# BioinfoMachineLearning/bio-diffusion

Hardware: NVIDIA H100
Metric: molecules/sec (1000-step sample) (higher is better)
Workload: dtype bf16x2 (split hi+lo operands, f32 accumulate; <=1e-4 of the fp32 reference)

## Files before the change

bio-diffusion_b200/csrc/bdiff_layers_tc.cu:

```cuda
#include "bdiff_node_tc.cuh"

namespace bdiff {

__device__ __forceinline__ int ld_acquire_gpu(const int* p) {
  int v;
  asm volatile("ld.acquire.gpu.global.s32 %0, [%1];" : "=r"(v) : "l"(p) : "memory");
  return v;
}
__device__ __forceinline__ void st_release_gpu(int* p, int v) {
  asm volatile("st.release.gpu.global.s32 [%0], %1;" ::"l"(p), "r"(v) : "memory");
}

union LayersTail {
  TcBars bars;
  EdgeTail edge;
  NodeTail node;
};
constexpr size_t LAYERS_SMEM_BYTES = XE_BLOCKS * (size_t)X_BLOCK + TC_NSLOT * (size_t)TC_SLOT + sizeof(LayersTail) + 1024;
static_assert(LAYERS_SMEM_BYTES + 64 <= 232448, "shared memory budget of the layer megakernel (227 KiB per block)");

constexpr int LAYERS_THREADS = 384;
constexpr int LAYERS_REG_COMPUTE = 232, LAYERS_REG_SERVICE = 40;
static_assert(256 * LAYERS_REG_COMPUTE + 128 * LAYERS_REG_SERVICE <= 168 * LAYERS_THREADS, "setmaxnreg pool");
constexpr int RING_CONSUMERS = TC_EPI / 32;

template <int NS, int NU, class Issue>
__device__ __forceinline__ void run_seg(TcBars& B, uint32_t raddr, uint32_t& ci, int nch, int scol, bool sfresh, int ucol,
                                        bool ufresh, Issue&& issue) {
  constexpr int RS = NS ? NS / 2 : 1, RU = NU ? NU / 2 : 1;
  const int wg = threadIdx.x >> 7;
  const bool lead = (threadIdx.x & 31) == 0;
  for (int h = 0; h < 2; ++h) {
    float s[RS], u[RU];
    if (NS) {
      if (sfresh) {
#pragma unroll
        for (int i = 0; i < RS; ++i) s[i] = 0.f;
      } else {
        acc_load<NS>(s, scol + h * NS, wg);
      }
    }
    if (NU) {
      if (ufresh) {
#pragma unroll
        for (int i = 0; i < RU; ++i) u[i] = 0.f;
      } else {
        acc_load<NU>(u, ucol + h * NU, wg);
      }
    }
    for (int c = 0; c < nch; ++c) {
      const uint32_t slot = ci % TC_NSLOT;
      float ts[RS], tu[RU];
#pragma unroll
      for (int i = 0; i < RS; ++i) ts[i] = 0.f;
#pragma unroll
      for (int i = 0; i < RU; ++i) tu[i] = 0.f;
      mbar_wait(&B.full[slot], (ci / TC_NSLOT) & 1);
      wgmma_fence();
      issue(ts, tu, raddr + slot * TC_SLOT, c);
      wgmma_commit();
      wgmma_wait<0>();
      acc_fence<RS>(ts);
      acc_fence<RU>(tu);
      mbar_arrive_if(&B.empty[slot], lead);
      ++ci;
      if (NS) {
#pragma unroll
        for (int i = 0; i < RS; ++i) s[i] += ts[i];
      }
      if (NU) {
#pragma unroll
        for (int i = 0; i < RU; ++i) u[i] += tu[i];
      }
    }
    if (NS) acc_store<NS>(s, scol + h * NS, wg);
    if (NU) acc_store<NU>(u, ucol + h * NU, wg);
  }
}

template <int ED, int XD>
__global__ void __launch_bounds__(LAYERS_THREADS, 1) k_layers_tc(Plan p, Dims d, EmbedW ew, LayerSched q, Work w) {
  constexpr int HID0 = (64 + XD) / 4;
  constexpr int H2 = HID0 / 2;
  constexpr int K0RAW = ED + HID0 + 9;
  constexpr int K0S = (K0RAW + 15) / 16;
  static_assert(HID0 % 2 == 0 && H2 * 3 <= 32 && HID0 + 9 <= 32 && ED % 16 == 0, "layout");

  extern __shared__ unsigned char smem_raw[];
  unsigned char* smem = smem_raw + ((1024u - (smem_u32(smem_raw) & 1023u)) & 1023u);
  unsigned char* X = smem;
  unsigned char* ring = smem + XE_BLOCKS * X_BLOCK;
  unsigned char* tail = ring + TC_NSLOT * TC_SLOT;
  TcBars& B = *reinterpret_cast<TcBars*>(tail);
  const int tid = threadIdx.x, warp = __shfl_sync(0xffffffffu, tid >> 5, 0), lane = tid & 31;
  const int hid0 = d.hid0;
  const int per_layer = q.TE + q.TN;
  const int total_items = q.nitems;
  int* const flags = q.sched + 2;

  if (tid == 0) {
    for (int i = 0; i < TC_NSLOT; ++i) { mbar_init(&B.full[i], 1); mbar_init(&B.empty[i], RING_CONSUMERS); }
    for (int i = 0; i < 2; ++i) { mbar_init(&B.item_full[i], 1); mbar_init(&B.item_empty[i], TC_EPI + 1); }
    mbar_init(&B.tile_done, TC_EPI);
    mbar_init(&B.wbar, 1);
    mbar_fence_init();
    tm_base = w.acc + (size_t)blockIdx.x * TM_COLS * 128;
  }
  __syncthreads();

  if (warp == 8) {
    asm volatile("setmaxnreg.dec.sync.aligned.u32 %0;\n" ::"n"(LAYERS_REG_SERVICE));
    if (lane == 0) {
      uint32_t ci = 0;
      for (uint32_t k = 0;; ++k) {
        const uint32_t slot = k & 1;
        mbar_wait_backoff(&B.item_empty[slot], ((k >> 1) & 1) ^ 1);
        int type = -1, layer = 0, tile = 0;
        for (;;) {
          const int qi = atomicAdd(q.sched, 1);
          if (qi >= 2 * total_items) break;
          const int it = __ldg(q.items + (qi >> 1));
          type = (it >> 30) & 1; layer = (it >> 24) & 63; tile = 2 * (it & 0xffffff) + (qi & 1);
          if (tile < (type == 0 ? q.TE : q.TN)) break;
          type = -1;
        }
        B.item[slot][0] = type; B.item[slot][1] = layer; B.item[slot][2] = tile;
        mbar_arrive(&B.item_full[slot]);
        if (type < 0) break;
        const size_t stride = type == 0 ? q.edge_blob_stride : q.node_blob_stride;
// ... 87 lines not shown
            cp(s.wgp, lw.Wgp, 256); cp(s.bgp, lw.bgp, 1);
            if (!last) {
              cp(s.u.nx.b0, wn.b0, 256);
              cp(s.u.nx.Wd0i, wn.Wd0i, 32 * hid0); cp(s.u.nx.Wd0j, wn.Wd0j, 32 * hid0);
              cp(s.u.nx.Wf0i, wn.Wf0i, 96); cp(s.u.nx.Wf0j, wn.Wf0j, 96);
            } else {
              cp(s.u.pj.pWd, ew.pWd, 32 * 32); cp(s.u.pj.pWf, ew.pWf, 96); cp(s.u.pj.pbs, ew.pbs, d.Hin);
            }
          }
        }
        mbar_wait(&B.wbar, pw);
        pw ^= 1;
        cur_type = type; cur_layer = layer;
      }
      if (tid == 0) {
        int lo = 0, hi = -1;
        const int* fbase = flags;
        if (type == 0) {
          if (layer > 0) {
            const int2 dep = q.edge_dep[tile];
            lo = dep.x; hi = dep.y;
            fbase = flags + (size_t)(layer - 1) * per_layer + q.TE;
          }
        } else {
          const int2 dep = q.node_dep[tile];
          lo = dep.x; hi = dep.y;
          fbase = flags + (size_t)layer * per_layer;
        }
        const long long t0 = clock64();
        for (int u = lo; u <= hi; ++u) {
          while (ld_acquire_gpu(fbase + u) == 0) {
            if (clock64() - t0 > (1ll << 32)) { atomicExch(q.err, 1); __threadfence_system(); __trap(); }
          }
        }
      }
      named_bar_sync(3, TC_EPI);
      __threadfence();
      if (tid == 0 && w.dbg && k < 16) w.dbg[(size_t)blockIdx.x * 64 + 4 * k + 2] = clock64();
      es = 0;
      stamp = nullptr;
      if (w.dbg && k >= 2 && !stamped[type]) { stamp = w.dbg + 256 * 64 + (size_t)blockIdx.x * 64 + type * 32; stamped[type] = true; }
      PH();
      const int last = type == 1 && layer == q.L - 1;
      int ph = 0;
      auto gemm = [&](int phase) __attribute__((always_inline)) {
        if (type == 0) {
          const int ph = phase;
#include "edge_tile_mma.inc"
        } else {
          const int ph = phase;
#include "node_r4_tile_mma.inc"
        }
      };
      auto publish = [&]() __attribute__((always_inline)) { fence_proxy_async(); named_bar_sync(3, TC_EPI); PH(); gemm(ph++); named_bar_sync(3, TC_EPI); PH(); };
      auto wait_d = [&]() __attribute__((always_inline)) {};
      auto release_u = [&]() __attribute__((always_inline)) { named_bar_sync(3, TC_EPI); gemm(-1); named_bar_sync(3, TC_EPI); };
      if (type == 0) {
        EdgeTail& T = *reinterpret_cast<EdgeTail*>(tail);
        const int half = tid >> 7, r = tid & 127;
        const SmallW& sw = T.sw;
        (void)release_u;
#include "edge_tile_epilogue.inc"
      } else {
        NodeTail& T = *reinterpret_cast<NodeTail*>(tail);
        NodeScratch& SC = *reinterpret_cast<NodeScratch*>(X + R5_BLOCKS * R5_BLOCK);
        const int l = lane, s = warp, c0 = warp * 32;
        const SmallWR4& sw = T.sw;
        (void)T;
#include "node_r4_tile_epilogue.inc"
      }
      PH();
      if (tid == 0 && w.dbg && k < 16) w.dbg[(size_t)blockIdx.x * 64 + 4 * k + 3] = clock64();
      mbar_arrive(&B.tile_done);
      mbar_arrive(&B.item_empty[slot]);
    }
  }
  __syncthreads();
}

bool tc_supported(int Ed, int Xd) { return (Ed == 64 && Xd == 16) || (Ed == 16 && Xd == 8); }

cudaError_t tc_layers_configure() {
  cudaError_t e = cudaFuncSetAttribute(k_layers_tc<64, 16>, cudaFuncAttributeMaxDynamicSharedMemorySize,
                                       (int)LAYERS_SMEM_BYTES);
  if (e != cudaSuccess) return e;
  return cudaFuncSetAttribute(k_layers_tc<16, 8>, cudaFuncAttributeMaxDynamicSharedMemorySize, (int)LAYERS_SMEM_BYTES);
}

void launch_layers_tc(cudaStream_t st, const Plan& p, const Dims& d, const EmbedW& ew, const LayerSched& q,
                      const Work& w, int num_sms) {
  const int grid = 2 * q.nitems < num_sms ? 2 * q.nitems : num_sms;
  if (d.Ed == 64) k_layers_tc<64, 16><<<grid, LAYERS_THREADS, LAYERS_SMEM_BYTES, st>>>(p, d, ew, q, w);
  else k_layers_tc<16, 8><<<grid, LAYERS_THREADS, LAYERS_SMEM_BYTES, st>>>(p, d, ew, q, w);
}

}
```

bio-diffusion_b200/csrc/bdiff_tc.cuh:

```cuda
#pragma once
#include <cuda_bf16.h>
#include <stdint.h>

#include "bdiff_common.cuh"

namespace bdiff {

__device__ __forceinline__ uint32_t sw128_offset(int r, int k) {
  return (uint32_t)(r * 128 + ((((k >> 3) ^ (r & 7)) & 7) << 4) + (k & 7) * 2);
}

__device__ __forceinline__ uint64_t gmma_desc_sw128(uint32_t saddr) {
  uint64_t d = 0;
  d |= (uint64_t)((saddr >> 4) & 0x3FFF);
  d |= (uint64_t)1 << 16;
  d |= (uint64_t)((1024 >> 4) & 0x3FFF) << 32;
  d |= (uint64_t)1 << 62;
  return d;
}

__device__ __forceinline__ uint64_t gmma_desc_k16(uint32_t saddr, uint32_t lbo, uint32_t sbo) {
  uint64_t d = 0;
  d |= (uint64_t)((saddr >> 4) & 0x3FFF);
  d |= (uint64_t)((lbo >> 4) & 0x3FFF) << 16;
// ... 4 lines not shown
template <int SA>
__device__ __forceinline__ void wgmma_n128(float* d, uint64_t ad, uint64_t bd) {
  asm volatile(
      "{\n.reg .pred p;\nsetp.ne.b32 p, %66, 0;\n"
      "wgmma.mma_async.sync.aligned.m64n128k16.f32.bf16.bf16 "
      "{%0,%1,%2,%3,%4,%5,%6,%7,%8,%9,%10,%11,%12,%13,%14,%15,%16,%17,%18,%19,%20,%21,%22,%23,%24,%25,%26,%27,%28,%29,%30,%31,%32,%33,%34,%35,%36,%37,%38,%39,%40,%41,%42,%43,%44,%45,%46,%47,%48,%49,%50,%51,%52,%53,%54,%55,%56,%57,%58,%59,%60,%61,%62,%63}, %64, %65, p, %67, 1, 0, 0;\n}\n"
      : "+f"(d[0]), "+f"(d[1]), "+f"(d[2]), "+f"(d[3]), "+f"(d[4]), "+f"(d[5]), "+f"(d[6]), "+f"(d[7]), "+f"(d[8]), "+f"(d[9]), "+f"(d[10]), "+f"(d[11]), "+f"(d[12]), "+f"(d[13]), "+f"(d[14]), "+f"(d[15]), "+f"(d[16]), "+f"(d[17]), "+f"(d[18]), "+f"(d[19]), "+f"(d[20]), "+f"(d[21]), "+f"(d[22]), "+f"(d[23]), "+f"(d[24]), "+f"(d[25]), "+f"(d[26]), "+f"(d[27]), "+f"(d[28]), "+f"(d[29]), "+f"(d[30]), "+f"(d[31]), "+f"(d[32]), "+f"(d[33]), "+f"(d[34]), "+f"(d[35]), "+f"(d[36]), "+f"(d[37]), "+f"(d[38]), "+f"(d[39]), "+f"(d[40]), "+f"(d[41]), "+f"(d[42]), "+f"(d[43]), "+f"(d[44]), "+f"(d[45]), "+f"(d[46]), "+f"(d[47]), "+f"(d[48]), "+f"(d[49]), "+f"(d[50]), "+f"(d[51]), "+f"(d[52]), "+f"(d[53]), "+f"(d[54]), "+f"(d[55]), "+f"(d[56]), "+f"(d[57]), "+f"(d[58]), "+f"(d[59]), "+f"(d[60]), "+f"(d[61]), "+f"(d[62]), "+f"(d[63])
      : "l"(ad), "l"(bd), "r"(1), "n"(SA));
}

template <int SA>
__device__ __forceinline__ void wgmma_n32(float* d, uint64_t ad, uint64_t bd) {
  asm volatile(
      "{\n.reg .pred p;\nsetp.ne.b32 p, %18, 0;\n"
      "wgmma.mma_async.sync.aligned.m64n32k16.f32.bf16.bf16 "
      "{%0,%1,%2,%3,%4,%5,%6,%7,%8,%9,%10,%11,%12,%13,%14,%15}, %16, %17, p, %19, 1, 0, 0;\n}\n"
      : "+f"(d[0]), "+f"(d[1]), "+f"(d[2]), "+f"(d[3]), "+f"(d[4]), "+f"(d[5]), "+f"(d[6]), "+f"(d[7]), "+f"(d[8]), "+f"(d[9]), "+f"(d[10]), "+f"(d[11]), "+f"(d[12]), "+f"(d[13]), "+f"(d[14]), "+f"(d[15])
      : "l"(ad), "l"(bd), "r"(1), "n"(SA));
}

template <int SA>
__device__ __forceinline__ void wgmma_n16(float* d, uint64_t ad, uint64_t bd) {
  asm volatile(
      "{\n.reg .pred p;\nsetp.ne.b32 p, %10, 0;\n"
      "wgmma.mma_async.sync.aligned.m64n16k16.f32.bf16.bf16 "
      "{%0,%1,%2,%3,%4,%5,%6,%7}, %8, %9, p, %11, 1, 0, 0;\n}\n"
      : "+f"(d[0]), "+f"(d[1]), "+f"(d[2]), "+f"(d[3]), "+f"(d[4]), "+f"(d[5]), "+f"(d[6]), "+f"(d[7])
      : "l"(ad), "l"(bd), "r"(1), "n"(SA));
}

__device__ __forceinline__ void wgmma_fence() { asm volatile("wgmma.fence.sync.aligned;" ::: "memory"); }
__device__ __forceinline__ void wgmma_commit() { asm volatile("wgmma.commit_group.sync.aligned;" ::: "memory"); }
template <int N>
__device__ __forceinline__ void wgmma_wait() { asm volatile("wgmma.wait_group.sync.aligned %0;" ::"n"(N) : "memory"); }
template <int R>
__device__ __forceinline__ void acc_fence(float* d) {
#pragma unroll
  for (int i = 0; i < R; ++i) asm volatile("" : "+f"(d[i])::"memory");
}

__device__ __forceinline__ void fence_proxy_async() { asm volatile("fence.proxy.async.shared::cta;" ::: "memory"); }
__device__ __forceinline__ void mbar_arrive(uint64_t* bar) {
  asm volatile("mbarrier.arrive.shared::cta.b64 _, [%0];" ::"r"(smem_u32(bar)) : "memory");
}
__device__ __forceinline__ void mbar_arrive_if(uint64_t* bar, bool pred) {
  asm volatile("{\n.reg .pred p;\nsetp.ne.b32 p, %1, 0;\n@p mbarrier.arrive.shared::cta.b64 _, [%0];\n}\n" ::"r"(smem_u32(bar)),
               "r"((int)pred) : "memory");
}

__shared__ float* tm_base;
__device__ __forceinline__ float* tm_word(uint32_t taddr) {
  return tm_base + (size_t)(taddr & 0xffffu) * 128 + (taddr >> 16) + (threadIdx.x & 31);
}
template <int N>
__device__ __forceinline__ void acc_store(const float* d, int col0, int wg) {
  const int lane = threadIdx.x & 31, row = 64 * wg + 16 * ((threadIdx.x >> 5) & 3) + (lane >> 2);
#pragma unroll
  for (int j = 0; j < N / 2; ++j)
    tm_base[(size_t)(col0 + 8 * (j >> 2) + 2 * (lane & 3) + (j & 1)) * 128 + row + 8 * ((j >> 1) & 1)] = d[j];
}
template <int N>
__device__ __forceinline__ void acc_load(float* d, int col0, int wg) {
  const int lane = threadIdx.x & 31, row = 64 * wg + 16 * ((threadIdx.x >> 5) & 3) + (lane >> 2);
#pragma unroll
  for (int j = 0; j < N / 2; ++j)
    d[j] = tm_base[(size_t)(col0 + 8 * (j >> 2) + 2 * (lane & 3) + (j & 1)) * 128 + row + 8 * ((j >> 1) & 1)];
}

__device__ __forceinline__ void tmem_ld8_nw(uint32_t taddr, uint32_t* r) {
  const float* p = tm_word(taddr);
#pragma unroll
  for (int i = 0; i < 8; ++i) r[i] = __float_as_uint(p[i * 128]);
}
__device__ __forceinline__ void tmem_ld32_nw(uint32_t taddr, uint32_t* r) {
  const float* p = tm_word(taddr);
#pragma unroll
  for (int i = 0; i < 32; ++i) r[i] = __float_as_uint(p[i * 128]);
}
__device__ __forceinline__ void tmem_ld_wait() {}
__device__ __forceinline__ void tmem_ld8(uint32_t taddr, float* v) {
  const float* p = tm_word(taddr);
#pragma unroll
  for (int i = 0; i < 8; ++i) v[i] = p[i * 128];
}
__device__ __forceinline__ void tmem_ld32(uint32_t taddr, float* v) {
  const float* p = tm_word(taddr);
#pragma unroll
  for (int i = 0; i < 32; ++i) v[i] = p[i * 128];
}
__device__ __forceinline__ void tmem_st8_nw(uint32_t taddr, const float* v) {
  float* p = tm_word(taddr);
#pragma unroll
  for (int i = 0; i < 8; ++i) p[i * 128] = v[i];
}
__device__ __forceinline__ void tmem_st_wait() {}
template <int N8>
__device__ __forceinline__ void tmem_ld8xN(uint32_t taddr, float* v) {
  const float* p = tm_word(taddr);
#pragma unroll
  for (int i = 0; i < N8 * 8; ++i) v[i] = p[i * 128];
}
template <int N8>
__device__ __forceinline__ void tmem_st8xN(uint32_t taddr, const float* v) {
#pragma unroll
  for (int q = 0; q < N8; ++q) tmem_st8_nw(taddr + q * 8, v + q * 8);
}
__device__ __forceinline__ void tmem_ld64(uint32_t taddr, float* v) { tmem_ld8xN<8>(taddr, v); }
__device__ __forceinline__ void tmem_st8(uint32_t taddr, const float* v) { tmem_st8_nw(taddr, v); }
__device__ __forceinline__ void tc_fence_before() {}
__device__ __forceinline__ void tc_fence_after() {}

#if defined(__CUDA_ARCH__) && __CUDA_ARCH__ < 1000
__device__ __forceinline__ float2 __fmul2_rn(float2 a, float2 b) { return make_float2(a.x * b.x, a.y * b.y); }
__device__ __forceinline__ float2 __fadd2_rn(float2 a, float2 b) { return make_float2(a.x + b.x, a.y + b.y); }
__device__ __forceinline__ float2 __ffma2_rn(float2 a, float2 b, float2 c) { return make_float2(fmaf(a.x, b.x, c.x), fmaf(a.y, b.y, c.y)); }
#endif

__device__ __forceinline__ float tanh_fast(float x) {
  float y;
// ... 77 lines not shown
```

bio-diffusion_b200/csrc/edge_tile_epilogue.inc:

```
      const long long g = (long long)tile * TMT + r;
      constexpr int PV = HID0 * 3 + 9, PF4 = (PV + 3) / 4, PLD = PF4 * 4 + 1;
      constexpr int XF4 = XD * 3 / 4, XLD = XD * 3 + 1;
      static_assert(K0S <= 8 && TMT * XLD * 4 <= 2 * X_BLOCK && TMT * PLD * 4 <= 3 * X_BLOCK, "staging areas");
      float* sFx = reinterpret_cast<float*>(X + 2 * X_BLOCK);
      float* sFp = reinterpret_cast<float*>(X + 6 * X_BLOCK);
      const int4 rc = __ldg(p.edge_rc + g);
      float f[9];
      {
        constexpr int F4_ROW = ED / 4;
        const float4* eb = reinterpret_cast<const float4*>(w.e + (size_t)tile * TMT * ED);
        const float4* xb = reinterpret_cast<const float4*>(w.xi + (size_t)tile * TMT * XD * 3);
        float4 ev[TMT * F4_ROW / TC_EPI], xv[TMT * XF4 / TC_EPI];
#pragma unroll
        for (int i = 0; i < TMT * F4_ROW / TC_EPI; ++i) ev[i] = eb[i * TC_EPI + tid];
#pragma unroll
        for (int i = 0; i < TMT * XF4 / TC_EPI; ++i) xv[i] = xb[i * TC_EPI + tid];
#pragma unroll
        for (int qq = 0; qq < 9; ++qq) f[qq] = w.frames[(size_t)g * 9 + qq];
        if (half == 0) { T.sRow[r] = rc.x; T.sCol[r] = rc.y; T.sB[r] = rc.z; T.sNa[r] = rc.w; }
#pragma unroll
        for (int i = 0; i < TMT * F4_ROW / TC_EPI; ++i) {
          const int idx = i * TC_EPI + tid;
          const int rr = idx / F4_ROW, kk = (idx % F4_ROW) * 4;
          xe_store4(X, rr, kk, ev[i].x, ev[i].y, ev[i].z, ev[i].w);
        }
#pragma unroll
        for (int i = 0; i < TMT * XF4 / TC_EPI; ++i) {
          const int idx = i * TC_EPI + tid;
          float* dst = sFx + (idx / XF4) * XLD + (idx % XF4) * 4;
          dst[0] = xv[i].x; dst[1] = xv[i].y; dst[2] = xv[i].z; dst[3] = xv[i].w;
        }
      }
      const int row = rc.x;
      const float* pi = w.PI + (size_t)(row < 0 ? 0 : row) * kPStride;
      named_bar_sync(3, TC_EPI);
      {
        float4 pv[(TMT * PF4 + TC_EPI - 1) / TC_EPI];
#pragma unroll
        for (int i = 0; i < (TMT * PF4 + TC_EPI - 1) / TC_EPI; ++i) {
          const int idx = i * TC_EPI + tid;
          pv[i] = make_float4(0.f, 0.f, 0.f, 0.f);
          if (idx < TMT * PF4) {
            const int rr = idx / PF4, cj = T.sCol[rr];
            if (cj >= 0) pv[i] = *reinterpret_cast<const float4*>(w.PJ + (size_t)cj * kPStride + kH + (idx - rr * PF4) * 4);
          }
        }
        float vdh[32], vdf0[9];
#pragma unroll
        for (int i = 0; i < 32; ++i) vdh[i] = 0.f;
#pragma unroll
        for (int i = 0; i < 9; ++i) vdf0[i] = 0.f;
        if (row >= 0) {
#pragma unroll
          for (int i = 0; i < H2 * 3; ++i) vdh[i] = pi[kH + half * H2 * 3 + i];
          if (half == 0) {
#pragma unroll
            for (int i = 0; i < 9; ++i) vdf0[i] = pi[kH + HID0 * 3 + i];
          }
        }
        float xi[XD * 3];
#pragma unroll
        for (int c = 0; c < XD * 3; ++c) xi[c] = sFx[r * XLD + c];
#pragma unroll
        for (int i = 0; i < (TMT * PF4 + TC_EPI - 1) / TC_EPI; ++i) {
          const int idx = i * TC_EPI + tid;
          if (idx < TMT * PF4) {
            const int rr = idx / PF4;
            float* dst = sFp + rr * PLD + (idx - rr * PF4) * 4;
            dst[0] = pv[i].x; dst[1] = pv[i].y; dst[2] = pv[i].z; dst[3] = pv[i].w;
          }
        }
        named_bar_sync(3, TC_EPI);
        const float* pjv = sFp + r * PLD;
#pragma unroll
        for (int i = 0; i < H2 * 3; ++i) vdh[i] += pjv[half * H2 * 3 + i];
        if (half == 0) {
#pragma unroll
          for (int i = 0; i < 9; ++i) vdf0[i] += pjv[HID0 * 3 + i];
        }
#pragma unroll
        for (int c = 0; c < XD; ++c) {
#pragma unroll
          for (int h = 0; h < H2; ++h) {
            const float wd = sw.Wd0x[c * HID0 + half * H2 + h];
            vdh[h * 3 + 0] = fmaf(wd, xi[c * 3 + 0], vdh[h * 3 + 0]);
            vdh[h * 3 + 1] = fmaf(wd, xi[c * 3 + 1], vdh[h * 3 + 1]);
            vdh[h * 3 + 2] = fmaf(wd, xi[c * 3 + 2], vdh[h * 3 + 2]);
          }
        }
#pragma unroll
        for (int h = 0; h < H2; ++h)
          xe_store1(X, r, ED + half * H2 + h, safe_norm3(vdh[h * 3], vdh[h * 3 + 1], vdh[h * 3 + 2]));
        tmem_st8xN<4>(tl + TM_VD0 + half * 32, vdh);
        tmem_st_wait();
        if (half == 0) {
#pragma unroll
          for (int c = 0; c < XD; ++c)
#pragma unroll
            for (int ch = 0; ch < 3; ++ch) {
              const float wf = sw.Wf0x[c * 3 + ch];
              vdf0[ch * 3 + 0] = fmaf(wf, xi[c * 3 + 0], vdf0[ch * 3 + 0]);
              vdf0[ch * 3 + 1] = fmaf(wf, xi[c * 3 + 1], vdf0[ch * 3 + 1]);
              vdf0[ch * 3 + 2] = fmaf(wf, xi[c * 3 + 2], vdf0[ch * 3 + 2]);
            }
#pragma unroll
          for (int ch = 0; ch < 3; ++ch)
#pragma unroll
            for (int ax = 0; ax < 3; ++ax)
              xe_store1(X, r, ED + HID0 + ch * 3 + ax,
                        f[ax * 3] * vdf0[ch * 3] + f[ax * 3 + 1] * vdf0[ch * 3 + 1] + f[ax * 3 + 2] * vdf0[ch * 3 + 2]);
#pragma unroll
          for (int i = HID0 + 9; i < K0S * 16 - ED; ++i) xe_store1(X, r, ED + i, 0.f);
        }
      }
      publish();

      {
        float4 pa[8];
        float pj[32];
        const int colj = rc.y;
        const int cjn = colj < 0 ? 0 : colj;
        const float* pjt = w.PJT + ((size_t)(cjn >> 5) * 256 + half * 128) * 32 + (cjn & 31);
        auto prefetch = [&](int c) {
          const float* pc = pjt + c * 1024;
#pragma unroll
          for (int i = 0; i < 32; ++i) pj[i] = pc[i * 32];
#pragma unroll
          for (int qq = 0; qq < 8; ++qq) pa[qq] = *reinterpret_cast<const float4*>(pi + half * 128 + c * 32 + qq * 4);
        };
        prefetch(0);
        wait_d();
        for (int c = 0; c < 4; ++c) {
          const int c0 = half * 128 + c * 32;
          float v[32];
          tmem_ld32(tl + TM_S + c0, v);
#pragma unroll
          for (int qq = 0; qq < 8; ++qq) {
            v[qq * 4 + 0] += pa[qq].x + pj[qq * 4 + 0]; v[qq * 4 + 1] += pa[qq].y + pj[qq * 4 + 1];
            v[qq * 4 + 2] += pa[qq].z + pj[qq * 4 + 2]; v[qq * 4 + 3] += pa[qq].w + pj[qq * 4 + 3];
          }
          if (c < 3) prefetch(c + 1);
#pragma unroll
          for (int qq = 0; qq < 16; ++qq) {
            const float2 p0 = silu_acc2(make_float2(v[2 * qq], v[2 * qq + 1]));
            v[2 * qq] = p0.x; v[2 * qq + 1] = p0.y;
          }
#pragma unroll
          for (int qq = 0; qq < 4; ++qq) xe_store8(X, r, c0 + qq * 8, v + qq * 8);
        }
      }
      publish();

      float vd[24], vdf[9];
      float2 adot2 = make_float2(0.f, 0.f);
      for (int k = 1; k <= 3; ++k) {
        wait_d();
        float part[33], other[33];
        if (k == 1) {
          float vd0[HID0 * 3];
          {
            float t0[64];
            float* t1 = t0 + 32;
            tmem_ld64(tl + TM_VD0, t0);
#pragma unroll
            for (int i = 0; i < H2 * 3; ++i) { vd0[i] = t0[i]; vd0[H2 * 3 + i] = t1[i]; }
          }
          tc_fence_before();
          named_bar_sync(3, TC_EPI);
          tc_fence_after();
          gate_update<HID0, true, false>(tl, half, TM_U0, vd0, sw.Wu0, sw.bg[0], sw.Wdk[0], sw.Wfk[0], part);
        } else {
          gate_update<8, false, false>(tl, half, ((k - 1) & 1) ? TM_U1 : TM_U0, vd, sw.Wuk[k - 2], sw.bg[k - 1],
                                       sw.Wdk[k - 1], sw.Wfk[k - 1], part);
        }
        pair_exchange33(tl, half, part, other);
#pragma unroll
        for (int i = 0; i < 24; ++i) vd[i] = half == 0 ? part[i] + other[i] : other[i] + part[i];
#pragma unroll
        for (int i = 0; i < 9; ++i) vdf[i] = half == 0 ? part[24 + i] + other[24 + i] : other[24 + i] + part[24 + i];
        {
          float a[16];
          if (half == 0) {
#pragma unroll
            for (int h = 0; h < 8; ++h) a[h] = safe_norm3(vd[h * 3], vd[h * 3 + 1], vd[h * 3 + 2]);
#pragma unroll
            for (int i = 0; i < 8; ++i) {
              const int ch = i / 3, ax = i - ch * 3;
              a[8 + i] = f[ax * 3] * vdf[ch * 3] + f[ax * 3 + 1] * vdf[ch * 3 + 1] + f[ax * 3 + 2] * vdf[ch * 3 + 2];
            }
          } else {
            a[0] = f[6] * vdf[6] + f[7] * vdf[7] + f[8] * vdf[8];
#pragma unroll
            for (int i = 1; i < 16; ++i) a[i] = 0.f;
          }
          xe_store8_extra(X, r, half * 16, a);
          xe_store8_extra(X, r, half * 16 + 8, a + 8);
        }
        publish();
        wait_d();
        if (k < 3 && half == 0) {
          float z[32];
#pragma unroll
          for (int i = 0; i < 32; ++i) z[i] = 0.f;
          tmem_st8xN<4>(tl + (((k + 1) & 1) ? TM_U1 : TM_U0), z);
          tmem_st_wait();
        }
        for (int c0 = half * 128; c0 < half * 128 + 128; c0 += 64) {
          float v[64];
          tmem_ld64(tl + TM_S + c0, v);
#pragma unroll
          for (int qq = 0; qq < 8; ++qq) {
            float m[8];
            xe_load8(X, r, c0 + qq * 8, m);
            const float4 b0 = *reinterpret_cast<const float4*>(&sw.bk[k - 1][c0 + qq * 8]);
            const float4 b1 = *reinterpret_cast<const float4*>(&sw.bk[k - 1][c0 + qq * 8 + 4]);
            const float2 bb[4] = {make_float2(b0.x, b0.y), make_float2(b0.z, b0.w), make_float2(b1.x, b1.y),
                                  make_float2(b1.z, b1.w)};
            float2 mm[4];
#pragma unroll
            for (int i = 0; i < 4; ++i)
              mm[i] = __fadd2_rn(make_float2(m[2 * i], m[2 * i + 1]),
                                 silu_acc2(__fadd2_rn(make_float2(v[qq * 8 + 2 * i], v[qq * 8 + 2 * i + 1]), bb[i])));
#pragma unroll
            for (int i = 0; i < 4; ++i) { m[2 * i] = mm[i].x; m[2 * i + 1] = mm[i].y; }
            xe_store8(X, r, c0 + qq * 8, m);
            if (k == 3) {
              const float4 w0 = *reinterpret_cast<const float4*>(&sw.wa[c0 + qq * 8]);
              const float4 w1 = *reinterpret_cast<const float4*>(&sw.wa[c0 + qq * 8 + 4]);
              adot2 = __ffma2_rn(mm[0], make_float2(w0.x, w0.y), adot2);
              adot2 = __ffma2_rn(mm[1], make_float2(w0.z, w0.w), adot2);
              adot2 = __ffma2_rn(mm[2], make_float2(w1.x, w1.y), adot2);
              adot2 = __ffma2_rn(mm[3], make_float2(w1.z, w1.w), adot2);
            }
          }
        }
        if (k == 3) T.sAttn[half][r] = adot2.x + adot2.y;
        publish();
      }
      const int wr0 = warp * 16;
      uint32_t m_start, m_end;
      {
        const int li = lane & 15, tr = wr0 + li;
        const int rw = T.sRow[tr];
        const int rp = tr > 0 ? T.sRow[tr - 1] : -2;
        const int rn = tr < TMT - 1 ? T.sRow[tr + 1] : -2;
        m_start = __ballot_sync(0xffffffffu, rw != rp) & 0xffffu;
        m_end = __ballot_sync(0xffffffffu, rw != rn && rw >= 0) & 0xffffu;
        if (lane == 0) T.winfo[warp] = m_start | (m_end << 16);
      }
      named_bar_sync(3, TC_EPI);
      const bool cutL = T.sB[0] != 0;
      const bool cutR = T.sRow[TMT - 1] >= 0 && T.sB[TMT - 1] != T.sNa[TMT - 1] - 1;
      const bool cont_in = !(m_start & 1u);
      float attw[16];
#pragma unroll
      for (int i = 0; i < 16; ++i) attw[i] = sigmoid_acc(T.sAttn[0][wr0 + i] + T.sAttn[1][wr0 + i] + sw.ba[0]);
      auto emit = [&](int trow, float2 val, int t, bool active) {
        if (!active) return;
        const bool l = cutL && (T.sRow[trow] == T.sRow[0]);
        const bool rr_ = cutR && (T.sRow[trow] == T.sRow[TMT - 1]);
        const size_t col = (size_t)t * 64 + 2 * lane;
        if (l && rr_) *reinterpret_cast<float2*>(w.mid + (size_t)tile * kMsg + col) = val;
        else if (l || rr_) atomicAdd(reinterpret_cast<float2*>(w.agg + (size_t)T.sRow[trow] * kMsg + col), val);
        else *reinterpret_cast<float2*>(w.agg + (size_t)T.sRow[trow] * kMsg + col) = val;
      };
      auto finish_crossing = [&](int t, bool active) {
        if (!(cont_in && (m_end & 0xffffu))) return;
        const float2 (*wb)[2][32] = T.wbuf[t & 1];
        int wa = warp - 1;
        while (wa > 0 && !(T.winfo[wa] & 0xffffu) && !(T.winfo[wa] >> 16)) --wa;
        float2 s = wb[wa][1][lane];
        for (int v2 = wa + 1; v2 < warp; ++v2) s = __fadd2_rn(s, wb[v2][1][lane]);
        s = __fadd2_rn(s, wb[warp][0][lane]);
        emit(wr0 + (__ffs(m_end & 0xffffu) - 1), s, t, active);
      };
      for (int t = 0; t < 4; ++t) {
        const unsigned char* xh_ = X + t * X_BLOCK + (lane & 3) * 4;
        const unsigned char* xl_ = X + (XE_LO + t) * X_BLOCK + (lane & 3) * 4;
        float2 acc = make_float2(0.f, 0.f);
        bool from_prev = cont_in;
        uint32_t hw[16], lw_[16];
#pragma unroll
        for (int i = 0; i < 16; ++i) {
          const int row_ = wr0 + i;
          const uint32_t off = (uint32_t)row_ * 128u + ((((uint32_t)lane >> 2) ^ ((uint32_t)row_ & 7u)) << 4);
          hw[i] = *reinterpret_cast<const uint32_t*>(xh_ + off);
          lw_[i] = *reinterpret_cast<const uint32_t*>(xl_ + off);
        }
#pragma unroll
// ... 66 lines not shown
```

bio-diffusion_b200/csrc/edge_tile_mma.inc:

```
        {
          auto adh = [&](int ks) { return gmma_desc_sw128(xa + (ks >> 2) * X_BLOCK + (ks & 3) * 32); };
          auto adl = [&](int ks) { return gmma_desc_sw128(xa + (XE_LO + (ks >> 2)) * X_BLOCK + (ks & 3) * 32); };
          auto bd = [](uint32_t b, int nl) { return gmma_desc_k16(b, nl * 16, 128); };
          if (ph == 0) {
            run_seg<128, 0>(B, raddr, ci, K0S, TM_S, true, 0, false, [&](float* s, float*, uint32_t wb, int ks) {
              const uint64_t h = bd(wb, 128), l = bd(wb + 128 * 32, 128);
              wgmma_n128<1>(s, adh(ks), h); wgmma_n128<1>(s, adl(ks), h); wgmma_n128<1>(s, adh(ks), l);
            });
          } else if (ph == 7) {
            run_seg<0, 16>(B, raddr, ci, 4, 0, false, TM_U1, false, [&](float*, float* u, uint32_t wb, int c) {
#pragma unroll
              for (int s4 = 0; s4 < 4; ++s4) {
                const int ks = c * 4 + s4;
                const uint64_t h = bd(wb + s4 * 1024, 16), l = bd(wb + s4 * 1024 + 512, 16);
                wgmma_n16<1>(u, adh(ks), h); wgmma_n16<1>(u, adl(ks), h); wgmma_n16<1>(u, adh(ks), l);
              }
            });
          } else if (ph & 1) {
            const int k = (ph + 1) >> 1;
            run_seg<128, 32>(B, raddr, ci, 16, TM_S, true, TM_U0, k == 1, [&](float* s, float* u, uint32_t wb, int ks) {
              const uint32_t bl = wb + 160 * 32;
              const uint64_t ah = adh(ks), al = adl(ks);
              wgmma_n128<1>(s, ah, bd(wb, 160)); wgmma_n32<1>(u, ah, bd(wb + 128 * 16, 160));
              wgmma_n128<1>(s, al, bd(wb, 160)); wgmma_n32<1>(u, al, bd(wb + 128 * 16, 160));
              wgmma_n128<1>(s, ah, bd(bl, 160)); wgmma_n32<1>(u, ah, bd(bl + 128 * 16, 160));
            });
          } else {
            const uint32_t xe = xa + XE_EXTRA * X_BLOCK;
            run_seg<128, 0>(B, raddr, ci, 2, TM_S, false, 0, false, [&](float* s, float*, uint32_t wb, int ks) {
              const uint64_t ah = gmma_desc_sw128(xe + ks * 32), al = gmma_desc_sw128(xe + 64 + ks * 32);
              const uint64_t h = bd(wb, 128), l = bd(wb + 128 * 32, 128);
              wgmma_n128<1>(s, ah, h); wgmma_n128<1>(s, al, h); wgmma_n128<1>(s, ah, l);
            });
          }
        }
```

bio-diffusion_b200/csrc/node_r4_tile_mma.inc:

```
        {
          auto bd = [](uint32_t b, int nl) { return gmma_desc_k16(b, nl * 16, 128); };
          auto v0 = [&](int ks) { return gmma_desc_sw128(xa + (ks >> 2) * R5_BLOCK + (ks & 3) * 32); };
          auto v1 = [&](int ks) { return gmma_desc_sw128(xa + (ks >> 2) * R5_BLOCK + 4096 + (ks & 3) * 32); };
          auto ngemm = [&](int nl, int dcol, bool fresh, int umode) {
            if (umode) {
              run_seg<128, 16>(B, raddr, ci, 16, dcol, fresh, NM_U, umode == 2, [&](float* s, float* u, uint32_t wb, int ks) {
                const uint64_t a0 = v0(ks), a1 = v1(ks);
#pragma unroll
                for (int pl = 0; pl < 2; ++pl) {
                  const uint32_t b = wb + pl * nl * 32;
                  wgmma_n128<1>(s, a0, bd(b, nl)); wgmma_n128<1>(s, a1, bd(b, nl));
                  wgmma_n16<1>(u, a0, bd(b + 128 * 16, nl)); wgmma_n16<1>(u, a1, bd(b + 128 * 16, nl));
                }
              });
            } else {
              run_seg<128, 0>(B, raddr, ci, 16, dcol, fresh, 0, false, [&](float* s, float*, uint32_t wb, int ks) {
                const uint64_t a0 = v0(ks), a1 = v1(ks);
#pragma unroll
                for (int pl = 0; pl < 2; ++pl) {
                  const uint32_t b = wb + pl * nl * 32;
                  wgmma_n128<1>(s, a0, bd(b, nl)); wgmma_n128<1>(s, a1, bd(b, nl));
                }
              });
            }
          };
          auto nextra = [&]() {
            run_seg<128, 0>(B, raddr, ci, 2, NM_S, false, 0, false, [&](float* s, float*, uint32_t wb, int ks) {
              const uint32_t a = xa + 4 * R5_BLOCK + ks * 32;
              const uint64_t a0 = gmma_desc_sw128(a), a1 = gmma_desc_sw128(a + 4096);
#pragma unroll
              for (int pl = 0; pl < 2; ++pl) {
                const uint64_t b = bd(wb + pl * 128 * 32, 128);
                wgmma_n128<1>(s, a0, b); wgmma_n128<1>(s, a1, b);
              }
            });
          };
          if (ph == -1) ngemm(128, NM_S1, true, 0);
          else if (ph == 0) ngemm(128, NM_S, true, 0);
          else if (ph == 1) { ngemm(144, NM_S, false, 2); nextra(); }
          else if (ph == 2) ngemm(128, NM_S, true, 0);
          else if (ph == 3) ngemm(144, NM_S, true, 1);
          else if (ph == 4) nextra();
          else if (!last) ngemm(128, NM_S, true, 0);
          else {
            run_seg<0, 16>(B, raddr, ci, 5, 0, false, NM_U, true, [&](float*, float* u, uint32_t wb, int c) {
              const int ns = c < 4 ? 4 : 3;
              for (int s4 = 0; s4 < ns; ++s4) {
                const int ks = c * 4 + s4;
                const uint64_t a0 = v0(ks), a1 = v1(ks);
                const uint64_t bh = bd(wb + s4 * 1024, 16), bl = bd(wb + s4 * 1024 + 512, 16);
                wgmma_n16<1>(u, a0, bh); wgmma_n16<1>(u, a1, bh); wgmma_n16<1>(u, a0, bl); wgmma_n16<1>(u, a1, bl);
              }
            });
          }
        }
```

Measured before the change: 21.98.

## Fuse edge GEMM epilogues into wgmma register accumulators, skipping scratch round-trip

Adds an optional register-level epilogue to run_seg so the edge-tile GEMM results are consumed directly from the wgmma accumulator fragments, instead of being written to scratch and reloaded by a separate epilogue pass. The first edge GEMM now applies the PI/PJT bias, SiLU and bf16 hi/lo split straight into the A operand, and the message-update GEMMs fuse the bias, SiLU, residual add and the attention dot product with shuffles. This removes scratch stores, loads and barriers between phases, and moves the staging buffers to a column offset. In exchange it adds scattered global loads keyed by fragment row and more register pressure in the compute warps. The ufresh flag becomes a per-half bitmask, and zeroing of the U accumulators is handled inside the GEMM.

```diff
diff --git a/bio-diffusion_b200/csrc/bdiff_layers_tc.cu b/bio-diffusion_b200/csrc/bdiff_layers_tc.cu
--- a/bio-diffusion_b200/csrc/bdiff_layers_tc.cu
+++ b/bio-diffusion_b200/csrc/bdiff_layers_tc.cu
@@ -1,3 +1,5 @@
+#include <type_traits>
+
 #include "bdiff_node_tc.cuh"
 
 namespace bdiff {
@@ -24,9 +26,10 @@
 static_assert(256 * LAYERS_REG_COMPUTE + 128 * LAYERS_REG_SERVICE <= 168 * LAYERS_THREADS, "setmaxnreg pool");
 constexpr int RING_CONSUMERS = TC_EPI / 32;
 
-template <int NS, int NU, class Issue>
+struct AccToScratch {};
+template <int NS, int NU, class Issue, class Epi = AccToScratch>
 __device__ __forceinline__ void run_seg(TcBars& B, uint32_t raddr, uint32_t& ci, int nch, int scol, bool sfresh, int ucol,
-                                        bool ufresh, Issue&& issue) {
+                                        int ufresh, Issue&& issue, Epi&& epi = Epi{}) {
   constexpr int RS = NS ? NS / 2 : 1, RU = NU ? NU / 2 : 1;
   const int wg = threadIdx.x >> 7;
   const bool lead = (threadIdx.x & 31) == 0;
@@ -41,7 +44,7 @@
       }
     }
     if (NU) {
-      if (ufresh) {
+      if ((ufresh >> h) & 1) {
 #pragma unroll
         for (int i = 0; i < RU; ++i) u[i] = 0.f;
       } else {
@@ -73,8 +76,12 @@
         for (int i = 0; i < RU; ++i) u[i] += tu[i];
       }
     }
-    if (NS) acc_store<NS>(s, scol + h * NS, wg);
-    if (NU) acc_store<NU>(u, ucol + h * NU, wg);
+    if constexpr (std::is_same_v<std::decay_t<Epi>, AccToScratch>) {
+      if (NS) acc_store<NS>(s, scol + h * NS, wg);
+      if (NU) acc_store<NU>(u, ucol + h * NU, wg);
+    } else {
+      epi(s, u, h, wg);
+    }
   }
 }
 
@@ -268,7 +275,8 @@
 #include "node_r4_tile_mma.inc"
         }
       };
-      auto publish = [&]() __attribute__((always_inline)) { fence_proxy_async(); named_bar_sync(3, TC_EPI); PH(); gemm(ph++); named_bar_sync(3, TC_EPI); PH(); };
+      auto run = [&]() __attribute__((always_inline)) { fence_proxy_async(); named_bar_sync(3, TC_EPI); PH(); gemm(ph++); };
+      auto publish = [&]() __attribute__((always_inline)) { run(); named_bar_sync(3, TC_EPI); PH(); };
       auto wait_d = [&]() __attribute__((always_inline)) {};
       auto release_u = [&]() __attribute__((always_inline)) { named_bar_sync(3, TC_EPI); gemm(-1); named_bar_sync(3, TC_EPI); };
       if (type == 0) {
@@ -283,6 +291,7 @@
         const int l = lane, s = warp, c0 = warp * 32;
         const SmallWR4& sw = T.sw;
         (void)T;
+        (void)run;
 #include "node_r4_tile_epilogue.inc"
       }
       PH();
diff --git a/bio-diffusion_b200/csrc/bdiff_tc.cuh b/bio-diffusion_b200/csrc/bdiff_tc.cuh
--- a/bio-diffusion_b200/csrc/bdiff_tc.cuh
+++ b/bio-diffusion_b200/csrc/bdiff_tc.cuh
@@ -80,19 +80,21 @@
 __device__ __forceinline__ float* tm_word(uint32_t taddr) {
   return tm_base + (size_t)(taddr & 0xffffu) * 128 + (taddr >> 16) + (threadIdx.x & 31);
 }
+__device__ __forceinline__ int frag_row(int wg, int j) {
+  return 64 * wg + 16 * ((threadIdx.x >> 5) & 3) + ((threadIdx.x & 31) >> 2) + 8 * ((j >> 1) & 1);
+}
+__device__ __forceinline__ int frag_col(int j) { return 8 * (j >> 2) + 2 * (threadIdx.x & 3) + (j & 1); }
 template <int N>
 __device__ __forceinline__ void acc_store(const float* d, int col0, int wg) {
-  const int lane = threadIdx.x & 31, row = 64 * wg + 16 * ((threadIdx.x >> 5) & 3) + (lane >> 2);
-#pragma unroll
-  for (int j = 0; j < N / 2; ++j)
-    tm_base[(size_t)(col0 + 8 * (j >> 2) + 2 * (lane & 3) + (j & 1)) * 128 + row + 8 * ((j >> 1) & 1)] = d[j];
+  float* const base = tm_base;
+#pragma unroll
+  for (int j = 0; j < N / 2; ++j) base[(size_t)(col0 + frag_col(j)) * 128 + frag_row(wg, j)] = d[j];
 }
 template <int N>
 __device__ __forceinline__ void acc_load(float* d, int col0, int wg) {
-  const int lane = threadIdx.x & 31, row = 64 * wg + 16 * ((threadIdx.x >> 5) & 3) + (lane >> 2);
-#pragma unroll
-  for (int j = 0; j < N / 2; ++j)
-    d[j] = tm_base[(size_t)(col0 + 8 * (j >> 2) + 2 * (lane & 3) + (j & 1)) * 128 + row + 8 * ((j >> 1) & 1)];
+  const float* const base = tm_base;
+#pragma unroll
+  for (int j = 0; j < N / 2; ++j) d[j] = base[(size_t)(col0 + frag_col(j)) * 128 + frag_row(wg, j)];
 }
 
 __device__ __forceinline__ void tmem_ld8_nw(uint32_t taddr, uint32_t* r) {
diff --git a/bio-diffusion_b200/csrc/edge_tile_epilogue.inc b/bio-diffusion_b200/csrc/edge_tile_epilogue.inc
--- a/bio-diffusion_b200/csrc/edge_tile_epilogue.inc
+++ b/bio-diffusion_b200/csrc/edge_tile_epilogue.inc
@@ -1,9 +1,10 @@
       const long long g = (long long)tile * TMT + r;
       constexpr int PV = HID0 * 3 + 9, PF4 = (PV + 3) / 4, PLD = PF4 * 4 + 1;
       constexpr int XF4 = XD * 3 / 4, XLD = XD * 3 + 1;
-      static_assert(K0S <= 8 && TMT * XLD * 4 <= 2 * X_BLOCK && TMT * PLD * 4 <= 3 * X_BLOCK, "staging areas");
-      float* sFx = reinterpret_cast<float*>(X + 2 * X_BLOCK);
-      float* sFp = reinterpret_cast<float*>(X + 6 * X_BLOCK);
+      constexpr int C0 = 128;
+      static_assert(K0S <= 8 && 64 * (PLD + XLD) * 4 <= 2 * X_BLOCK, "staging areas");
+      auto sFp = [&](int rr) { return reinterpret_cast<float*>(X + (rr >> 6) * XE_LO * X_BLOCK) + (rr & 63) * PLD; };
+      auto sFx = [&](int rr) { return reinterpret_cast<float*>(X + (rr >> 6) * XE_LO * X_BLOCK) + 64 * PLD + (rr & 63) * XLD; };
       const int4 rc = __ldg(p.edge_rc + g);
       float f[9];
       {
@@ -22,12 +23,12 @@
         for (int i = 0; i < TMT * F4_ROW / TC_EPI; ++i) {
           const int idx = i * TC_EPI + tid;
           const int rr = idx / F4_ROW, kk = (idx % F4_ROW) * 4;
-          xe_store4(X, rr, kk, ev[i].x, ev[i].y, ev[i].z, ev[i].w);
+          xe_store4(X, rr, C0 + kk, ev[i].x, ev[i].y, ev[i].z, ev[i].w);
         }
 #pragma unroll
         for (int i = 0; i < TMT * XF4 / TC_EPI; ++i) {
           const int idx = i * TC_EPI + tid;
-          float* dst = sFx + (idx / XF4) * XLD + (idx % XF4) * 4;
+          float* dst = sFx(idx / XF4) + (idx % XF4) * 4;
           dst[0] = xv[i].x; dst[1] = xv[i].y; dst[2] = xv[i].z; dst[3] = xv[i].w;
         }
       }
@@ -60,18 +61,18 @@
         }
         float xi[XD * 3];
 #pragma unroll
-        for (int c = 0; c < XD * 3; ++c) xi[c] = sFx[r * XLD + c];
+        for (int c = 0; c < XD * 3; ++c) xi[c] = sFx(r)[c];
 #pragma unroll
         for (int i = 0; i < (TMT * PF4 + TC_EPI - 1) / TC_EPI; ++i) {
           const int idx = i * TC_EPI + tid;
           if (idx < TMT * PF4) {
             const int rr = idx / PF4;
-            float* dst = sFp + rr * PLD + (idx - rr * PF4) * 4;
+            float* dst = sFp(rr) + (idx - rr * PF4) * 4;
             dst[0] = pv[i].x; dst[1] = pv[i].y; dst[2] = pv[i].z; dst[3] = pv[i].w;
           }
         }
         named_bar_sync(3, TC_EPI);
-        const float* pjv = sFp + r * PLD;
+        const float* pjv = sFp(r);
 #pragma unroll
         for (int i = 0; i < H2 * 3; ++i) vdh[i] += pjv[half * H2 * 3 + i];
         if (half == 0) {
@@ -90,7 +91,7 @@
         }
 #pragma unroll
         for (int h = 0; h < H2; ++h)
-          xe_store1(X, r, ED + half * H2 + h, safe_norm3(vdh[h * 3], vdh[h * 3 + 1], vdh[h * 3 + 2]));
+          xe_store1(X, r, C0 + ED + half * H2 + h, safe_norm3(vdh[h * 3], vdh[h * 3 + 1], vdh[h * 3 + 2]));
         tmem_st8xN<4>(tl + TM_VD0 + half * 32, vdh);
         tmem_st_wait();
         if (half == 0) {
@@ -107,52 +108,16 @@
           for (int ch = 0; ch < 3; ++ch)
 #pragma unroll
             for (int ax = 0; ax < 3; ++ax)
-              xe_store1(X, r, ED + HID0 + ch * 3 + ax,
+              xe_store1(X, r, C0 + ED + HID0 + ch * 3 + ax,
                         f[ax * 3] * vdf0[ch * 3] + f[ax * 3 + 1] * vdf0[ch * 3 + 1] + f[ax * 3 + 2] * vdf0[ch * 3 + 2]);
 #pragma unroll
-          for (int i = HID0 + 9; i < K0S * 16 - ED; ++i) xe_store1(X, r, ED + i, 0.f);
-        }
-      }
-      publish();
-
-      {
-        float4 pa[8];
-        float pj[32];
-        const int colj = rc.y;
-        const int cjn = colj < 0 ? 0 : colj;
-        const float* pjt = w.PJT + ((size_t)(cjn >> 5) * 256 + half * 128) * 32 + (cjn & 31);
-        auto prefetch = [&](int c) {
-          const float* pc = pjt + c * 1024;
-#pragma unroll
-          for (int i = 0; i < 32; ++i) pj[i] = pc[i * 32];
-#pragma unroll
-          for (int qq = 0; qq < 8; ++qq) pa[qq] = *reinterpret_cast<const float4*>(pi + half * 128 + c * 32 + qq * 4);
-        };
-        prefetch(0);
-        wait_d();
-        for (int c = 0; c < 4; ++c) {
-          const int c0 = half * 128 + c * 32;
-          float v[32];
-          tmem_ld32(tl + TM_S + c0, v);
-#pragma unroll
-          for (int qq = 0; qq < 8; ++qq) {
-            v[qq * 4 + 0] += pa[qq].x + pj[qq * 4 + 0]; v[qq * 4 + 1] += pa[qq].y + pj[qq * 4 + 1];
-            v[qq * 4 + 2] += pa[qq].z + pj[qq * 4 + 2]; v[qq * 4 + 3] += pa[qq].w + pj[qq * 4 + 3];
-          }
-          if (c < 3) prefetch(c + 1);
-#pragma unroll
-          for (int qq = 0; qq < 16; ++qq) {
-            const float2 p0 = silu_acc2(make_float2(v[2 * qq], v[2 * qq + 1]));
-            v[2 * qq] = p0.x; v[2 * qq + 1] = p0.y;
-          }
-#pragma unroll
-          for (int qq = 0; qq < 4; ++qq) xe_store8(X, r, c0 + qq * 8, v + qq * 8);
-        }
-      }
+          for (int i = HID0 + 9; i < K0S * 16 - ED; ++i) xe_store1(X, r, C0 + ED + i, 0.f);
+        }
+      }
+      run();
       publish();
 
       float vd[24], vdf[9];
-      float2 adot2 = make_float2(0.f, 0.f);
       for (int k = 1; k <= 3; ++k) {
         wait_d();
         float part[33], other[33];
@@ -196,45 +161,7 @@
           xe_store8_extra(X, r, half * 16, a);
           xe_store8_extra(X, r, half * 16 + 8, a + 8);
         }
-        publish();
-        wait_d();
-        if (k < 3 && half == 0) {
-          float z[32];
-#pragma unroll
-          for (int i = 0; i < 32; ++i) z[i] = 0.f;
-          tmem_st8xN<4>(tl + (((k + 1) & 1) ? TM_U1 : TM_U0), z);
-          tmem_st_wait();
-        }
-        for (int c0 = half * 128; c0 < half * 128 + 128; c0 += 64) {
-          float v[64];
-          tmem_ld64(tl + TM_S + c0, v);
-#pragma unroll
-          for (int qq = 0; qq < 8; ++qq) {
-            float m[8];
-            xe_load8(X, r, c0 + qq * 8, m);
-            const float4 b0 = *reinterpret_cast<const float4*>(&sw.bk[k - 1][c0 + qq * 8]);
-            const float4 b1 = *reinterpret_cast<const float4*>(&sw.bk[k - 1][c0 + qq * 8 + 4]);
-            const float2 bb[4] = {make_float2(b0.x, b0.y), make_float2(b0.z, b0.w), make_float2(b1.x, b1.y),
-                                  make_float2(b1.z, b1.w)};
-            float2 mm[4];
-#pragma unroll
-            for (int i = 0; i < 4; ++i)
-              mm[i] = __fadd2_rn(make_float2(m[2 * i], m[2 * i + 1]),
-                                 silu_acc2(__fadd2_rn(make_float2(v[qq * 8 + 2 * i], v[qq * 8 + 2 * i + 1]), bb[i])));
-#pragma unroll
-            for (int i = 0; i < 4; ++i) { m[2 * i] = mm[i].x; m[2 * i + 1] = mm[i].y; }
-            xe_store8(X, r, c0 + qq * 8, m);
-            if (k == 3) {
-              const float4 w0 = *reinterpret_cast<const float4*>(&sw.wa[c0 + qq * 8]);
-              const float4 w1 = *reinterpret_cast<const float4*>(&sw.wa[c0 + qq * 8 + 4]);
-              adot2 = __ffma2_rn(mm[0], make_float2(w0.x, w0.y), adot2);
-              adot2 = __ffma2_rn(mm[1], make_float2(w0.z, w0.w), adot2);
-              adot2 = __ffma2_rn(mm[2], make_float2(w1.x, w1.y), adot2);
-              adot2 = __ffma2_rn(mm[3], make_float2(w1.z, w1.w), adot2);
-            }
-          }
-        }
-        if (k == 3) T.sAttn[half][r] = adot2.x + adot2.y;
+        run();
         publish();
       }
       const int wr0 = warp * 16;
diff --git a/bio-diffusion_b200/csrc/edge_tile_mma.inc b/bio-diffusion_b200/csrc/edge_tile_mma.inc
--- a/bio-diffusion_b200/csrc/edge_tile_mma.inc
+++ b/bio-diffusion_b200/csrc/edge_tile_mma.inc
@@ -2,13 +2,38 @@
           auto adh = [&](int ks) { return gmma_desc_sw128(xa + (ks >> 2) * X_BLOCK + (ks & 3) * 32); };
           auto adl = [&](int ks) { return gmma_desc_sw128(xa + (XE_LO + (ks >> 2)) * X_BLOCK + (ks & 3) * 32); };
           auto bd = [](uint32_t b, int nl) { return gmma_desc_k16(b, nl * 16, 128); };
+          EdgeTail& ET = *reinterpret_cast<EdgeTail*>(tail);
+          auto a_word = [&](int rr, int c) { return reinterpret_cast<uint32_t*>(X + (c >> 6) * X_BLOCK + sw128_offset(rr, c & 63)); };
           if (ph == 0) {
-            run_seg<128, 0>(B, raddr, ci, K0S, TM_S, true, 0, false, [&](float* s, float*, uint32_t wb, int ks) {
+            run_seg<128, 0>(B, raddr, ci, K0S, TM_S, true, 0, 0, [&](float* s, float*, uint32_t wb, int ks) {
               const uint64_t h = bd(wb, 128), l = bd(wb + 128 * 32, 128);
-              wgmma_n128<1>(s, adh(ks), h); wgmma_n128<1>(s, adl(ks), h); wgmma_n128<1>(s, adh(ks), l);
+              wgmma_n128<1>(s, adh(ks + 8), h); wgmma_n128<1>(s, adl(ks + 8), h); wgmma_n128<1>(s, adh(ks + 8), l);
+            }, [&](float* s, float*, int h, int wg) __attribute__((always_inline)) {
+              const float* pi[2];
+              const float* pj[2];
+#pragma unroll
+              for (int r8 = 0; r8 < 2; ++r8) {
+                const int rr = frag_row(wg, 2 * r8);
+                const int ri = ET.sRow[rr], cj = ET.sCol[rr];
+                const int rin = ri < 0 ? 0 : ri, cjn = cj < 0 ? 0 : cj;
+                pi[r8] = w.PI + (size_t)rin * kPStride + h * 128;
+                pj[r8] = w.PJT + ((size_t)(cjn >> 5) * 256 + h * 128) * 32 + (cjn & 31);
+              }
+#pragma unroll
+              for (int j = 0; j < 64; j += 2) {
+                const int r8 = (j >> 1) & 1, c = frag_col(j);
+                const float2 pa = *reinterpret_cast<const float2*>(pi[r8] + c);
+                const float v0 = s[j] + (pa.x + pj[r8][c * 32]), v1 = s[j + 1] + (pa.y + pj[r8][(c + 1) * 32]);
+                const float2 m = silu_acc2(make_float2(v0, v1));
+                const int rr = frag_row(wg, j), cc = h * 128 + c;
+                uint32_t hi, lo;
+                split_bf16x2(m.x, m.y, hi, lo);
+                a_word(rr, cc)[0] = hi;
+                a_word(rr, cc)[XE_LO * X_BLOCK / 4] = lo;
+              }
             });
           } else if (ph == 7) {
-            run_seg<0, 16>(B, raddr, ci, 4, 0, false, TM_U1, false, [&](float*, float* u, uint32_t wb, int c) {
+            run_seg<0, 16>(B, raddr, ci, 4, 0, false, TM_U1, 0, [&](float*, float* u, uint32_t wb, int c) {
 #pragma unroll
               for (int s4 = 0; s4 < 4; ++s4) {
                 const int ks = c * 4 + s4;
@@ -18,7 +43,7 @@
             });
           } else if (ph & 1) {
             const int k = (ph + 1) >> 1;
-            run_seg<128, 32>(B, raddr, ci, 16, TM_S, true, TM_U0, k == 1, [&](float* s, float* u, uint32_t wb, int ks) {
+            run_seg<128, 32>(B, raddr, ci, 16, TM_S, true, TM_U0, k == 1 ? 3 : 1 << (k & 1), [&](float* s, float* u, uint32_t wb, int ks) {
               const uint32_t bl = wb + 160 * 32;
               const uint64_t ah = adh(ks), al = adl(ks);
               wgmma_n128<1>(s, ah, bd(wb, 160)); wgmma_n32<1>(u, ah, bd(wb + 128 * 16, 160));
@@ -26,11 +51,47 @@
               wgmma_n128<1>(s, ah, bd(bl, 160)); wgmma_n32<1>(u, ah, bd(bl + 128 * 16, 160));
             });
           } else {
+            const int k = ph >> 1;
             const uint32_t xe = xa + XE_EXTRA * X_BLOCK;
-            run_seg<128, 0>(B, raddr, ci, 2, TM_S, false, 0, false, [&](float* s, float*, uint32_t wb, int ks) {
+            run_seg<128, 0>(B, raddr, ci, 2, TM_S, false, 0, 0, [&](float* s, float*, uint32_t wb, int ks) {
               const uint64_t ah = gmma_desc_sw128(xe + ks * 32), al = gmma_desc_sw128(xe + 64 + ks * 32);
               const uint64_t h = bd(wb, 128), l = bd(wb + 128 * 32, 128);
               wgmma_n128<1>(s, ah, h); wgmma_n128<1>(s, al, h); wgmma_n128<1>(s, ah, l);
+            }, [&](float* s, float*, int h, int wg) __attribute__((always_inline)) {
+              const float* bk = ET.sw.bk[k - 1] + h * 128;
+#pragma unroll
+              for (int j = 0; j < 64; j += 2) {
+                const int rr = frag_row(wg, j), c = frag_col(j);
+                uint32_t* wd = a_word(rr, h * 128 + c);
+                const float2 m = join_bf16x2(wd[0], wd[XE_LO * X_BLOCK / 4]);
+                const float2 mm = __fadd2_rn(m, silu_acc2(__fadd2_rn(make_float2(s[j], s[j + 1]),
+                                                                     *reinterpret_cast<const float2*>(bk + c))));
+                uint32_t hi, lo;
+                split_bf16x2(mm.x, mm.y, hi, lo);
+                wd[0] = hi;
+                wd[XE_LO * X_BLOCK / 4] = lo;
+                s[j] = mm.x; s[j + 1] = mm.y;
+              }
+              if (k == 3) {
+                const float* wa = ET.sw.wa + h * 128;
+                const int qb = threadIdx.x & 28;
+                float2 a[2] = {make_float2(0.f, 0.f), make_float2(0.f, 0.f)};
+#pragma unroll
+                for (int g = 0; g < 16; ++g) {
+                  const float2 wv = *reinterpret_cast<const float2*>(wa + frag_col(4 * g));
+#pragma unroll
+                  for (int q = 0; q < 4; ++q) {
+#pragma unroll
+                    for (int r8 = 0; r8 < 2; ++r8) {
+                      const int j = 4 * g + 2 * r8;
+                      const float2 t = __ffma2_rn(make_float2(s[j], s[j + 1]), wv, a[r8]);
+                      a[r8] = make_float2(__shfl_sync(0xffffffffu, t.x, qb | q), __shfl_sync(0xffffffffu, t.y, qb | q));
+                    }
+                  }
+                }
+                ET.sAttn[h][frag_row(wg, 0)] = a[0].x + a[0].y;
+                ET.sAttn[h][frag_row(wg, 2)] = a[1].x + a[1].y;
+              }
             });
           }
         }
diff --git a/bio-diffusion_b200/csrc/node_r4_tile_mma.inc b/bio-diffusion_b200/csrc/node_r4_tile_mma.inc
--- a/bio-diffusion_b200/csrc/node_r4_tile_mma.inc
+++ b/bio-diffusion_b200/csrc/node_r4_tile_mma.inc
@@ -4,7 +4,7 @@
           auto v1 = [&](int ks) { return gmma_desc_sw128(xa + (ks >> 2) * R5_BLOCK + 4096 + (ks & 3) * 32); };
           auto ngemm = [&](int nl, int dcol, bool fresh, int umode) {
             if (umode) {
-              run_seg<128, 16>(B, raddr, ci, 16, dcol, fresh, NM_U, umode == 2, [&](float* s, float* u, uint32_t wb, int ks) {
+              run_seg<128, 16>(B, raddr, ci, 16, dcol, fresh, NM_U, umode == 2 ? 3 : 0, [&](float* s, float* u, uint32_t wb, int ks) {
                 const uint64_t a0 = v0(ks), a1 = v1(ks);
 #pragma unroll
                 for (int pl = 0; pl < 2; ++pl) {
@@ -14,7 +14,7 @@
                 }
               });
             } else {
-              run_seg<128, 0>(B, raddr, ci, 16, dcol, fresh, 0, false, [&](float* s, float*, uint32_t wb, int ks) {
+              run_seg<128, 0>(B, raddr, ci, 16, dcol, fresh, 0, 0, [&](float* s, float*, uint32_t wb, int ks) {
                 const uint64_t a0 = v0(ks), a1 = v1(ks);
 #pragma unroll
                 for (int pl = 0; pl < 2; ++pl) {
@@ -25,7 +25,7 @@
             }
           };
           auto nextra = [&]() {
-            run_seg<128, 0>(B, raddr, ci, 2, NM_S, false, 0, false, [&](float* s, float*, uint32_t wb, int ks) {
+            run_seg<128, 0>(B, raddr, ci, 2, NM_S, false, 0, 0, [&](float* s, float*, uint32_t wb, int ks) {
               const uint32_t a = xa + 4 * R5_BLOCK + ks * 32;
               const uint64_t a0 = gmma_desc_sw128(a), a1 = gmma_desc_sw128(a + 4096);
 #pragma unroll
@@ -43,7 +43,7 @@
           else if (ph == 4) nextra();
           else if (!last) ngemm(128, NM_S, true, 0);
           else {
-            run_seg<0, 16>(B, raddr, ci, 5, 0, false, NM_U, true, [&](float*, float* u, uint32_t wb, int c) {
+            run_seg<0, 16>(B, raddr, ci, 5, 0, false, NM_U, 3, [&](float*, float* u, uint32_t wb, int c) {
               const int ns = c < 4 ? 4 : 3;
               for (int s4 = 0; s4 < ns; ++s4) {
                 const int ks = c * 4 + s4;
```

After: 23.36 (median of 6 runs). 1.06x the previous value.
